# thawro/pytorch-human-pose

Measured on AMD Instinct MI355X. Metric: images/sec (fwd+decode) HigherHRNet-W32 512px, higher is better.
Workload: dtype bf16; 1 GPU; HigherHRNet-W32 inference bf16, batch 32 @ 512x512 per GPU (conv fwd on N(0,1) images + AE decode on constructed maps, 10 people/image, det_thr 0.05, tag_thr 0.5, adjust+refine); global_batch=32, parallelism=image-sharded replicas x1, no data-path collective

## Files before the change

### include/hhrnet.h

```cpp
#ifndef HHRNET_H
#define HHRNET_H
#include <stdint.h>

#ifdef __cplusplus
extern "C" {
#endif

#define HH_ABI_VERSION 3
#define HH_DTYPE_BF16 1
#define HH_DTYPE_FP8 2

typedef struct hh_net hh_net;
typedef struct hh_decoder hh_decoder;

int hh_abi_version(void);
const char *hh_last_error(void);

hh_net *hh_create(int num_kpts, int C, int dtype);
void hh_destroy(hh_net *net);

hh_net *hh_create_classifier(int C, int num_classes, int dtype);
int hh_forward_classifier(hh_net *net, const float *images, int B, int H, int W, float *logits, void *stream);

int hh_num_params(const hh_net *net);
// ... 5 lines not shown

int hh_calibrate(hh_net *net, const float *images, int B, int H, int W, int rounds, void *stream);

int hh_e4m3_encode(const float *x, int64_t n, unsigned char *out);
int hh_e4m3_decode(const unsigned char *x, int64_t n, float *out);

int hh_reserve(hh_net *net, int B, int H, int W);
int64_t hh_workspace_bytes(const hh_net *net);

int hh_forward(hh_net *net, const float *images, int B, int H, int W, float *init_heatmaps, float *deconv_heatmaps,
               int use_graph, void *stream);

int hh_set_multi_lane(hh_net *net, int enable);

int hh_debug_check_plan(const hh_net *net);

double hh_forward_flops(const hh_net *net, int B, int H, int W);

int hh_profile_enable(hh_net *net, int enable);
int hh_profile_count(const hh_net *net);
int hh_profile_get(hh_net *net, int index, int *cfg, double *flops, double *bytes, float *ms, float *kernel_ms, const char **layer);
int hh_profile_clock(hh_net *net, int index, double *ghz);
int hh_conv_config(int cfg, int out[7]);
int hh_conv_config_double_buffered(int cfg);

int hh_debug_conv_bench(int cfg, int B, int Hin, int Win, int cin, int cout, int with_res, int relu, int iters,
                        float *ms_per_launch, unsigned long long *stamps16, int ref_cfg, float *max_diff);

int hh_debug_bb_bench(int B, int H, int W, int iters, float *ms_per_launch, unsigned long long *stamps64);
int hh_debug_bb_compare(int B, int H, int W, int iters, float *max_diff, float *ms_classic, float *ms_pc);
// ... 97 lines not shown
```

### pytorch-human-pose_amd/_lib.py

```python
from __future__ import annotations

import ctypes as C
import os
import subprocess

_HERE = os.path.dirname(os.path.abspath(__file__))
CSRC = os.path.join(_HERE, "csrc")
SO = os.environ.get("HH_LIB") or os.path.join(CSRC, "libhhrnet.so")
HEADER = os.path.join(os.path.dirname(_HERE), "include", "hhrnet.h")
_lib = None


class HHError(RuntimeError):
    pass


def build(force: bool = False, jobs: int = 8) -> str:
    args = ["make", "-C", CSRC, f"-j{jobs}"]
    if force:
        args.append("-B")
    subprocess.check_call(args, stdout=subprocess.DEVNULL)
    return SO


# ... 36 lines not shown
        "hh_debug_conv_bench": (i32, [i32, i32, i32, i32, i32, i32, i32, i32, i32, C.POINTER(C.c_float), vp, i32, C.POINTER(C.c_float)]),
        "hh_debug_bb_bench": (i32, [i32, i32, i32, i32, C.POINTER(C.c_float), vp]),
        "hh_debug_bb_compare": (i32, [i32, i32, i32, i32, C.POINTER(C.c_float), C.POINTER(C.c_float), C.POINTER(C.c_float)]),
        "hh_debug_bb_cover": (i32, [i32, i32, i32, i32, i32, pi64]),
        "hh_preprocess_u8": (i32, [vp, i32, i32, C.POINTER(C.c_double), vp, i32, i32, C.POINTER(C.c_float), C.POINTER(C.c_float), vp]),
        "hh_preprocess_u8_batch": (i32, [vp, vp, i32, vp, i32, i32, C.POINTER(C.c_float), C.POINTER(C.c_float), vp]),
        "hh_flip_images": (i32, [vp, vp, i32, i32, i32, i32, vp]),
        "hh_flip_merge": (i32, [vp, i64, vp, i64, vp, i64, vp, i64, vp, i32, i32, i32, i32, vp]),
        "hh_decoder_create": (vp, [i32, i32, dbl, dbl]),
        "hh_decoder_destroy": (None, [vp]),
        "hh_decoder_reserve": (i32, [vp, i32, i32, i32, i32]),
        "hh_decoder_set_exact_topk": (i32, [vp, i32]),
        "hh_decode": (i32, [vp, vp, i64, vp, i64, vp, pi64, i32, i32, i32, i32, i32, i32, vp, vp, vp, vp, vp]),
        "hh_parse": (i32, [vp, vp, vp, i32, i32, i32, i32, i32, i32, vp, vp, vp, vp, vp]),
        "hh_debug_check_plan": (i32, [vp]),
        "hh_loss_heatmaps": (i32, [vp, i64, vp, vp, i32, i32, i32, i32, vp, vp, i64, vp, vp]),
        "hh_loss_ae_grouping": (i32, [vp, i64, vp, vp, i32, i32, i32, i32, i32, vp, vp, i64, C.c_float, C.c_float, vp, vp]),
        "hh_conv2d_workspace_bytes": (i64, [i32, i32, i32, i32]),
        "hh_conv2d": (i32, [vp, i32, i32, i32, i32, vp, i32, i32, i32, i32, i32, i32, vp, vp, i32, vp, vp, vp]),
        "hh_conv2d_wgrad_workspace_bytes": (i64, [i32, i32, i32, i32, i32, i32, i32]),
        "hh_conv2d_wgrad": (i32, [vp, vp, i32, i32, i32, i32, i32, i32, i32, i32, i32, vp, vp, vp]),
        "hh_fusion_sum_forward": (i32, [vp, vp, i32, i32, i32, i32, i32, i32, vp, vp]),
        "hh_fusion_sum_backward": (i32, [vp, vp, i32, i32, i32, i32, i32, vp, vp, vp, i32, vp]),
        "hh_bn_train_forward": (i32, [vp, i64, i32, vp, vp, C.c_float, vp, i32, vp, vp, vp, vp, vp]),
        "hh_bn_train_backward": (i32, [vp, vp, vp, i64, i32, vp, vp, vp, i32, vp, vp, vp, vp, vp, vp]),
        "hh_bn_train_backward_plain": (i32, [vp, vp, i64, i32, vp, vp, vp, vp, i32, vp, vp, vp, vp, vp]),
        "hh_conv2d_packed_elems": (i64, [i32, i32, i32, i32, i32]),
        "hh_pack_conv_weights_batch": (i32, [i32, vp, vp, vp, vp, vp]),
        "hh_conv2d_packed": (i32, [vp, i32, i32, i32, i32, vp, i32, i32, i32, i32, i32, i32, vp, vp, i32, vp, vp]),
        "hh_bn_train_stats": (i32, [vp, i64, i32, vp, vp, vp]),
# ... 54 lines not shown
```

### pytorch-human-pose_amd/csrc/capi.cpp

```cpp
#include <cmath>
#include <cstring>
#include <string>
#include <vector>

#include "../../include/hhrnet.h"
#include "engine.h"

const char *hh_get_error();
int hh_tap_read_impl(hh_net *n, int index, float *host);

extern "C" {

int hh_abi_version(void) { return HH_ABI_VERSION; }
const char *hh_last_error(void) { return hh_get_error(); }

hh_net *hh_create(int num_kpts, int C, int dtype)
{
    if (dtype != HH_DTYPE_BF16 && dtype != HH_DTYPE_FP8) { hh_set_error("hh_create: dtype must be HH_DTYPE_BF16 or HH_DTYPE_FP8"); return nullptr; }
    if (num_kpts <= 0 || num_kpts > 64 || C <= 0 || C % 16) { hh_set_error("hh_create: need 0 < num_kpts <= 64 and C % 16 == 0"); return nullptr; }
    hh_net *n = new hh_net();
    n->K = num_kpts; n->C = C; n->dtype = dtype;
    n->sw = PlanSwitches::from_env();
    n->build();
    return n;
// ... 85 lines not shown
const char *hh_tap_name(const hh_net *net, int i) { return (i >= 0 && i < (int)net->taps.size()) ? net->taps[i].name.c_str() : nullptr; }
int hh_tap_shape(const hh_net *net, int i, int64_t shape[4])
{
    if (i < 0 || i >= (int)net->taps.size()) return 1;
    const TensorDesc &d = net->tensors[net->taps[i].tensor];
    shape[0] = net->lastB; shape[1] = net->taps[i].C; shape[2] = net->lastH >> d.shift; shape[3] = net->lastW >> d.shift;
    return 0;
}
int hh_tap_read(hh_net *net, int index, float *host_nchw) { return hh_tap_read_impl(net, index, host_nchw); }

int hh_debug_check_plan(const hh_net *net)
{
    std::string why;
    if (net->check_plan(&why)) { hh_set_error("schedule hazard: " + why); return 1; }
    return 0;
}

int hh_profile_enable(hh_net *net, int enable) { net->prof_enabled = enable != 0; net->prof_clk = enable == 2; net->prof_used = 0; return 0; }
int hh_profile_count(const hh_net *net) { return (int)net->prof_used; }
int hh_profile_get(hh_net *net, int i, int *cfg, double *flops, double *bytes, float *ms, float *kernel_ms, const char **layer)
{
    if (i < 0 || i >= (int)net->prof_used) { hh_set_error("hh_profile_get: index out of range"); return 1; }
    const ProfRecord &r = net->prof[i];
    HH_CHECK_HIP(hipEventSynchronize(r.e1));
    HH_CHECK_HIP(hipEventElapsedTime(ms, r.e0, r.e1));
    *cfg = r.cfg; *flops = r.flops; *bytes = r.bytes;
    *layer = net->layers[net->ops[r.op].layer].conv.c_str();
    *kernel_ms = -1.f;
    if (r.slot >= 0 && net->prof_clk && net->d_clk && net->clk_khz > 0) {
        unsigned long long t[2];
// ... 681 lines not shown
```

### pytorch-human-pose_amd/csrc/conv_mfma.hip

```cpp
#include "kernels.h"

#include <utility>

typedef __bf16 bf16x8 __attribute__((ext_vector_type(8)));
typedef __bf16 bf16x2 __attribute__((ext_vector_type(2)));
typedef float f32x16 __attribute__((ext_vector_type(16)));
typedef float f32x2 __attribute__((ext_vector_type(2)));
typedef unsigned u32x4 __attribute__((ext_vector_type(4)));

typedef short i16x2 __attribute__((ext_vector_type(2)));
__device__ __forceinline__ unsigned pack_bf16x2(float a, float b, i16x2 floor)
{
    f32x2 f = {a, b};
    const i16x2 v = __builtin_bit_cast(i16x2, __builtin_convertvector(f, bf16x2));
    return __builtin_bit_cast(unsigned, __builtin_elementwise_max(v, floor));
}
__device__ __forceinline__ float bf16_lo(unsigned u) { return __builtin_bit_cast(float, u << 16); }
__device__ __forceinline__ float bf16_hi(unsigned u) { return __builtin_bit_cast(float, u & 0xffff0000u); }

template <typename F, int... I>
__device__ __forceinline__ void static_for_impl(F &&f, std::integer_sequence<int, I...>)
{
    (f(std::integral_constant<int, I>{}), ...);
}
template <int N, typename F>
__device__ __forceinline__ void static_for(F &&f)
{
    static_for_impl(f, std::make_integer_sequence<int, N>{});
}

#ifdef HH_CONV_DEBUG
__device__ long long g_conv_dbg[8192 * 8];
#define CONV_STAMP(i) do { if (threadIdx.x == 0 && blockIdx.x < 8192) g_conv_dbg[blockIdx.x * 8 + (i)] = (long long)__builtin_readcyclecounter(); } while (0)
#else
#define CONV_STAMP(i)
#endif
template <int KS, int S, int KC, int NT, int WC, int PT, int TW, int DB>
__global__ __launch_bounds__(256, 2) void conv_mfma_kernel(const ConvParams p)
{
    constexpr int RPT = 32 / TW;
    constexpr int WP = 4 / WC;
    constexpr int TH = WP * PT * RPT;
    constexpr int PH = (TH - 1) * S + KS, PW = (TW - 1) * S + KS;
    constexpr int PS = KC * 2 + 16;
    constexpr int C8 = KC / 8;
    constexpr int COUT_T = 32 * NT * WC;
    constexpr int PATCH_BYTES = (PH * PW * PS + 15) & ~15;
    constexpr int P_UNITS = PH * PW * C8;
    constexpr int W_UNITS = KS * KS * C8 * COUT_T;
    constexpr int NPL = (P_UNITS + 255) / 256, NWL = (W_UNITS + 255) / 256, NL = NPL + NWL;
    constexpr int NSTEP = KS * KS * (KC / 16);
    constexpr int LPS = (NL + NSTEP - 1) / NSTEP;
    constexpr int DUMP_OFF = PATCH_BYTES + W_UNITS * 16;
    constexpr int BUF_BYTES = DUMP_OFF + (DB ? 256 * 16 : 0);
// ... 122 lines not shown
#pragma unroll
            for (int pt = 0; pt < PT; ++pt) {
                const int oy = oy0 + (wp * PT + pt) * RPT + dy, ox = ox0 + dx;
                const bool valid = oy < p.Ho && ox < p.Wo;
                const size_t pix = valid ? ((size_t)b * p.Hob + (oy * p.osy + ooy)) * p.Wob + (ox * p.osx + oox) : 0;
#pragma unroll
                for (int nt = 0; nt < NT; ++nt)
#pragma unroll
                    for (int m = 0; m < 2; ++m) {
                        const int c0 = cg * COUT_T + (wc * NT + nt) * 32 + 16 * m + 8 * h;
                        const bool ok = valid && c0 < p.cout_store;
                        const u32x4 v = *reinterpret_cast<const u32x4 *>(p.res + pix * p.res_cs + p.res_coff + (ok ? c0 : 0));
                        rv[pt][nt][m] = ok ? v : u32x4{0u, 0u, 0u, 0u};
                    }
            }
        }
#pragma unroll
        for (int pt = 0; pt < PT; ++pt)
#pragma unroll
            for (int nt = 0; nt < NT; ++nt)
#pragma unroll
                for (int m = 0; m < 2; ++m) {
                    unsigned x0 = 0, x1 = 0, y0 = 0, y1 = 0;
                    if (p.res) {
                        auto s0 = __builtin_amdgcn_permlane32_swap(rv[pt][nt][m][0], rv[pt][nt][m][2], false, false);
                        auto s1 = __builtin_amdgcn_permlane32_swap(rv[pt][nt][m][1], rv[pt][nt][m][3], false, false);
                        x0 = s0[0]; y0 = s0[1]; x1 = s1[0]; y1 = s1[1];
                    }
                    const float4 ba = bs[nt][2 * m], bb = bs[nt][2 * m + 1];
                    acc[nt][pt][8 * m + 0] = ba.x + bf16_lo(x0); acc[nt][pt][8 * m + 1] = ba.y + bf16_hi(x0);
// ... 216 lines not shown
    X(3, 1, 16, 2, 1, 2, 32, 1)  \
    X(3, 1, 16, 2, 1, 1, 16, 1)

#define CFG_ROW(ks, s, kc, nt, wc, pt, tw, db) {ks, s, kc, nt, wc, pt, tw, db},
static const ConvConfig g_configs[] = {CONV_CONFIGS(CFG_ROW)};
#undef CFG_ROW

typedef void (*conv_fn)(const ConvParams);
#define CFG_FN(ks, s, kc, nt, wc, pt, tw, db) conv_mfma_kernel<ks, s, kc, nt, wc, pt, tw, db>,
static const conv_fn g_fns[] = {CONV_CONFIGS(CFG_FN)};
#undef CFG_FN

int conv_num_configs() { return (int)(sizeof(g_configs) / sizeof(g_configs[0])); }
const ConvConfig &conv_config(int i) { return g_configs[i]; }

hipError_t conv_init()
{
    for (int i = 0; i < conv_num_configs(); ++i) {
        hipError_t e = hipFuncSetAttribute(reinterpret_cast<const void *>(g_fns[i]),
                                           hipFuncAttributeMaxDynamicSharedMemorySize, (int)g_configs[i].lds_bytes());
        if (e != hipSuccess) return e;
    }
    return hipSuccess;
}

hipError_t conv_launch(int cfg_index, const ConvParams &p, hipStream_t stream)
{
    const ConvConfig &c = g_configs[cfg_index];
    const unsigned tiles = (unsigned)p.B * p.tiles_y * p.tiles_x, sf = (unsigned)p.ncg * (p.nphase > 1 ? p.nphase : 1);
    const unsigned grid = sf > 1 ? (tiles + 7) / 8 * 8 * sf : tiles;
    HH_LAUNCH(g_fns[cfg_index], dim3(grid), dim3(256), c.lds_bytes(), stream, p);
    return hipGetLastError();
}
```

### pytorch-human-pose_amd/csrc/engine.cpp

```cpp
#include "engine.h"

#include <cmath>
#include <cstdlib>
#include <cstring>

static thread_local std::string g_err;
LaunchProbe &hh_launch_probe()
{
    static thread_local LaunchProbe p;
    return p;
}
void hh_set_error(const std::string &msg) { g_err = msg; }
const char *hh_get_error() { return g_err.c_str(); }

PlanSwitches PlanSwitches::from_env()
{
    auto on = [](const char *name) { const char *v = getenv(name); return v && *v && strcmp(v, "0"); };
    auto is = [](const char *name, const char *val) { const char *v = getenv(name); return v && !strcmp(v, val); };
    PlanSwitches s;
    s.bb32_tile = is("HH_BB32", "tile");
    s.no_bb64 = on("HH_NO_BB64");
    s.no_bb_fp8 = on("HH_NO_BB_FP8");
    s.no_stem_fused = on("HH_NO_STEM_FUSED");
    s.no_junc_pair = on("HH_NO_JUNC_PAIR");
    s.full_join = on("HH_FULL_JOIN");
    s.no_fusion_merge = on("HH_NO_FUSION_MERGE");
    s.no_fused_upsum = on("HH_NO_FUSED_UPSUM");
    s.poison_ws = on("HH_POISON_WS");
    s.poison_lds = on("HH_POISON_LDS");
    s.no_head_fold = on("HH_NO_HEAD_FOLD");
    s.no_conv_db = on("HH_NO_CONV_DB");
    s.no_final_fuse = on("HH_NO_FINAL_FUSE");
    s.keep_waits = on("HH_KEEP_WAITS");
    s.event_system_fence = on("HH_EVENT_SYSTEM_FENCE");
    s.bb_tall = on("HH_NO_BB_TALL") ? 0 : is("HH_BB_TALL", "always") ? 2 : 1;
    if (const char *fc = getenv("HH_FAT_CUS")) { s.fat_cus = s.fat_cus64 = atoi(fc); if (const char *c2 = strchr(fc, ',')) s.fat_cus64 = atoi(c2 + 1); }
    if (const char *sk = getenv("HH_DEBUG_SKIP")) {
        static const struct { const char *name; unsigned bit; } cats[] = {{"s2big", SK_S2BIG}, {"s2", SK_S2}, {"upadd", SK_UPADD}, {"c1x1", SK_C1X1},
            {"c256", SK_C256}, {"c128", SK_C128}, {"junc", SK_JUNC}, {"bb32", SK_BB32}, {"bb64", SK_BB64}, {"stem", SK_STEM}, {"deconv", SK_DECONV},
            {"head", SK_HEAD}, {"trans0", SK_TRANS0}, {"upsum", SK_UPSUM}};
        std::string v = std::string(",") + sk + ",";
        for (const auto &c : cats)
// ... 324 lines not shown
                    auto need_all = [&]() { for (int j = 0; j < nsc; ++j) need(j); };
                    if (i == 0 && n.dtype != 2 && w[0] == 32 && !n.sw.no_fused_upsum) {
                        Op o;
                        o.kind = OP_UPSUM; o.in = x[0]; o.out = OUT; o.C = w[0]; o.relu = 1; o.lane = lane;
                        for (int j = 1; j < nsc; ++j) {
                            const std::string lp = fp + ".scales_fusion_layers.0." + std::to_string(j);
                            o.up[o.nup] = x[j]; o.up_shift[o.nup] = j;
                            o.up_layer[o.nup] = L(lp + ".0", lp + ".1", w[j], w[0], 1, 1);
                            ++o.nup;
                        }
                        o.layer = o.up_layer[0];
                        need_all();
                        n.ops.push_back(o);
                        continue;
                    }
                    Op up;
                    up.kind = OP_UPADD; up.in = x[i]; up.out = OUT; up.C = w[i]; up.relu = (i == 0); up.lane = lane;
                    for (int j = i + 1; j < nsc; ++j) {
                        const std::string lp = fp + ".scales_fusion_layers." + std::to_string(i) + "." + std::to_string(j);
                        const int u = T(w[i], 2 + j);
                        need(j);
                        cb(lp, "0", "1", w[j], w[i], 1, 1, x[j], u, 0);
                        up.up[up.nup] = u; up.up_shift[up.nup] = j - i; ++up.nup;
                    }
                    if (up.nup) { need_all(); n.ops.push_back(up); cur = OUT; }
                    if (i >= 2 && n.dtype != 2 && !n.sw.no_fusion_merge) {
                        int srcs[3] = {-1, -1, -1};
                        ConvLayer ml;
                        ml.cout = w[i]; ml.ks = 3; ml.stride = 2; ml.cin = 0;
                        int tins[3] = {-1, -1, -1};
                        for (int j = 0; j < i; ++j) {
                            const std::string lp = fp + ".scales_fusion_layers." + std::to_string(i) + "." + std::to_string(j);
                            int tin = x[j];
// ... 7 lines not shown
                            tins[j] = tin;
                        }
                        for (int j = i - 1; j >= 0; --j) {
                            const std::string lp = fp + ".scales_fusion_layers." + std::to_string(i) + "." + std::to_string(j);
                            srcs[i - 1 - j] = tins[j];
                            ml.mconv.push_back(lp + "." + std::to_string(i - j - 1) + ".0");
                            ml.mbn.push_back(lp + "." + std::to_string(i - j - 1) + ".1");
                            ml.mcin.push_back(w[j]);
                            ml.cin += w[j];
                        }
                        ml.conv = ml.mconv[0]; ml.bn = ml.mbn[0];
                        n.layers.push_back(ml);
                        need_all();
                        Op &o = conv((int)n.layers.size() - 1, srcs[0], OUT, 1, cur);
                        o.in2 = srcs[1]; o.in3 = srcs[2];
                        cur = OUT;
                        continue;
                    }
                    for (int j = 0; j < i; ++j) {
                        const std::string lp = fp + ".scales_fusion_layers." + std::to_string(i) + "." + std::to_string(j);
                        int tin = x[j];
                        need(j);
                        for (int k = 0; k < i - j - 1; ++k) {
                            const int tmp = T(w[j], 2 + j + k + 1);
                            cb(lp + "." + std::to_string(k), "0", "1", w[j], w[j], 3, 2, tin, tmp, 1);
                            tin = tmp;
                        }
                        need_all();
                        cb(lp + "." + std::to_string(i - j - 1), "0", "1", w[j], w[i], 3, 2, tin, OUT, j == i - 1, cur);
                        cur = OUT;
                    }
                }
                lane = 0;
                if (!last)
                    for (int i = 0; i < nout; ++i) std::swap(x[i], f[i]);
                for (int i = 0; i < nout; ++i)
                    tap("stages." + std::to_string(s) + ".blocks." + std::to_string(2 * b + 1) + "#" + std::to_string(i),
                        last ? CAT : x[i], w[i]);
            }
            if (s < 3) {
                const std::string q = sp + ".transition_layer.transition_blocks." + std::to_string(nsc);
                x[nsc] = T(w[nsc], 2 + nsc);
                if (!n.sw.full_join) { mark(nsc + 1); waitl(nsc, nsc - 1); }
                else join(nsc + 1);
// ... 495 lines not shown
            const TensorDesc &ti = tensors[op.in];
            if (pool_cap < B * op.C) {
                if (d_pool) hipFree(d_pool);
                HH_CHECK_HIP(hipMalloc((void **)&d_pool, (size_t)B * op.C * 4));
                pool_cap = B * op.C;
            }
            HH_CHECK_HIP(launch_avgpool(ti.ptr, ti.C, d_pool, B, (H >> ti.shift) * (W >> ti.shift), op.C, s));
            break;
        }
        case OP_LINEAR:
            HH_CHECK_HIP(launch_linear(d_pool, d_fc_w, d_fc_b, o1, B, 2048, num_classes, s));
            break;
        case OP_STEM: rc = enqueue_stem(op, images, B, H, W, s); break;
        case OP_UPADD: rc = dtype == 2 ? enqueue_fp8_upadd(op, B, H, W, s) : enqueue_upadd(op, B, H, W, s); break;
        case OP_UPSUM: rc = enqueue_upsum(op, B, H, W, s); break;
        case OP_JUNC: rc = enqueue_junc(op, B, H, W, s); break;
        case OP_BB: rc = dtype == 2 ? enqueue_fp8_bb(op, B, H, W, s) : enqueue_bb(op, B, H, W, o2, multi, s, &fin_done); break;
        case OP_QUANT: rc = enqueue_fp8_quant(op, B, H, W, s); break;
        case OP_CONV: rc = dtype == 2 && !op.hi ? enqueue_fp8_conv(op, B, H, W, o1, o2, s) : enqueue_conv(op, B, H, W, o1, o2, s); break;
        }
        if (rc) return 1;
    }
    if (multi)
        for (int l = 1; l < lc.open; ++l)
            if ((lc.dep(0, l) || sw.keep_waits) && lane_wait(0, l)) return 1;
    return 0;
}

int hh_net::prof_record(const Op &op, int cfg, const OpCost &c, unsigned long long **clk)
{
// ... 112 lines not shown
        const ConvLayer &lf = layers[ops[op.fin].layer];
        p.fin_w = lf.d_wfin; p.fin_b = lf.d_bias; p.fin_out = o2; p.fin_K = lf.cout;
        if (lf.d_wfin && bbpc_final_supported(p)) *fin_done = op.fin;
        else { p.fin_w = nullptr; p.fin_b = nullptr; p.fin_out = nullptr; p.fin_K = 0; }
    }
    const int cfg = l1.cout == 64 ? HH_CFG_BB64_FUSED : HH_CFG_BB_FUSED;
    if (prof_enabled && prof_record(op, cfg, op_cost(op, B, H, W, p.fin_out != nullptr), &p.clk)) return 1;
    auto budget = [&](int want) { return !(multi && op.siblings) ? num_cus : want > 0 ? (want < num_cus ? want : num_cus) : (num_cus + 1) / 2; };
    const int fat = budget(sw.fat_cus), fat64 = budget(sw.fat_cus64);
    if (l1.cout == 64) HH_CHECK_HIP(bb64_fused_launch(p, fat64, s));
    else if (!sw.bb32_tile && bbpc_supported(p)) HH_CHECK_HIP(bbpc_launch(p, fat, s));
    else HH_CHECK_HIP(bb_fused_launch(p, num_cus, s));
    return 0;
}

int hh_net::enqueue_conv(const Op &op, int B, int H, int W, float *o1, float *o2, hipStream_t s)
{
    const ConvLayer &l = layers[op.layer];
    const TensorDesc &ti = tensors[op.in];
    ConvParams p{};
    hh_conv_geometry(p, l, op, B, H >> ti.shift, W >> ti.shift, o1, o2);
    p.in = dtype == 2 ? ti.ptr16 : ti.ptr; p.in_cs = ti.C; p.in_coff = op.in_coff;
    p.w = l.d_w; p.bias = l.d_bias;
    if (op.out >= 0) {
        const TensorDesc &to = tensors[op.out];
        p.out = dtype == 2 ? to.ptr16 : to.ptr; p.out_cs = to.C; p.out_coff = op.out_coff;
    }
    if (op.res >= 0) {
        const TensorDesc &tr = tensors[op.res];
        p.res = dtype == 2 ? tr.ptr16 : tr.ptr; p.res_cs = tr.C; p.res_coff = op.res_coff;
    }
    if (op.in2 >= 0) {
        const TensorDesc &t2 = tensors[op.in2];
        if (t2.C != ti.C || t2.shift != ti.shift || (op.in3 >= 0 && (tensors[op.in3].C != ti.C || tensors[op.in3].shift != ti.shift))) {
            hh_set_error("merged fusion conv: inputs differ in shape or pixel stride");
            return 1;
        }
        p.nch0 = l.mcin[0] / l.KC;
        p.nch1 = l.mcin[1] / l.KC;
        p.src_delta1 = t2.ptr - (ti.ptr + op.in_coff);
        if (op.in3 >= 0) p.src_delta2 = tensors[op.in3].ptr - (ti.ptr + op.in_coff);
    }
    p.cout_store = op.cout_store >= 0 ? op.cout_store : round_up(l.cout, 8);
    const int cfg = hh_pick_config(l.ks, l.stride, l.KC, l.NT, p.Wo, l.db);
    const ConvConfig &c = conv_config(cfg);
    p.tiles_x = (p.Wo + c.TW - 1) / c.TW;
    p.tiles_y = (p.Ho + c.th() - 1) / c.th();
    if (prof_enabled && prof_record(op, cfg, op_cost(op, B, H, W), &p.clk)) return 1;
    HH_CHECK_HIP(conv_launch(cfg, p, s));
    return 0;
}

int hh_net::forward(const float *images, int B, int H, int W, float *o1, float *o2, int use_graph, hipStream_t s)
{
    if (!finalized) { hh_set_error("hh_forward: call hh_finalize first"); return 1; }
    if (dtype == 2 && !calibrated) { hh_set_error("hh_forward: fp8 handle without activation scales, call hh_calibrate first"); return 1; }
    if (B > rB || H > rH || W > rW || !ws_ready || (taps_enabled && !taps.empty() && !taps[0].copy))
        if (reserve(B, H, W)) return 1;
    lastB = B; lastH = H; lastW = W;
    if (!use_graph || s == nullptr || taps_enabled || prof_enabled || sw.poison_lds || sw.debug_skip || multi_lane)
        return enqueue(images, B, H, W, o1, o2, s);
    for (auto &g : graphs)
        if (g.images == images && g.o1 == o1 && g.o2 == o2 && g.B == B && g.H == H && g.W == W) {
            HH_CHECK_HIP(hipGraphLaunch(g.exec, s));
// ... 28 lines not shown
    for (size_t i = 0; i < ops.size(); ++i) {
        const Op &op = ops[i];
        if (op.kind == OP_JOIN) { lc.join(op.nlanes); continue; }
        if (op.kind == OP_DEP) { lc.dep(op.lane, op.dep_from); continue; }
        if (op.kind == OP_MARK) { lc.set_mark(op.dep_from, op.nlanes); continue; }
        if (op.kind == OP_WAITL) {
            if (!lc.marked[op.dep_from]) { if (why) *why = "op " + std::to_string(i) + " waits for a lane the last mark did not record"; return 1; }
            lc.wait_mark(op.lane, op.dep_from);
            continue;
        }
        const int l = op.lane;
        if (l >= lc.open) { if (why) *why = "op " + std::to_string(i) + " runs on a lane that was never forked"; return 1; }
        std::vector<int> rd, wr;
        switch (op.kind) {
        case OP_CONV: rd = {op.in, op.res, op.in2, op.in3}; wr = {op.out}; break;
        case OP_UPADD: case OP_UPSUM: rd = {op.in, op.up[0], op.up[1], op.up[2]}; wr = {op.out}; break;
        case OP_BB: rd = {op.in}; wr = {op.out}; break;
        case OP_JUNC: rd = {op.in, op.in2, op.res, op.in3}; wr = {op.out, op.out2}; break;
        case OP_STEM: wr = {op.out}; break;
        case OP_QUANT: rd = {op.out}; wr = {op.out}; break;
        case OP_TAP: continue;
        case OP_AVGPOOL: rd = {op.in}; break;
        default: break;
        }
        const int t = lc.launch(l);
        for (int x : rd) {
            if (x < 0) continue;
            if (!before(writer[x], l)) {
                if (why) *why = "RAW: op " + std::to_string(i) + " (lane " + std::to_string(l) + ") reads tensor " + std::to_string(x) +
                                " written by op " + std::to_string(writer[x].op) + " (lane " + std::to_string(writer[x].lane) + ") without an edge";
// ... 53 lines not shown
    case OP_BB: {
        const TensorDesc &ti = tensors[op.in], &to = tensors[op.out];
        const double Cb = layers[op.layer].cout, npix = (double)B * (H >> ti.shift) * (W >> ti.shift);
        c.flops = 2.0 * 2.0 * npix * Cb * Cb * 9.0;
        if (dtype == 2)
            c.bytes = (2.0 + (ti.b16 ? 2.0 : 0.0) + (to.b16 ? 2.0 : 0.0)) * npix * Cb + 2.0 * 9 * Cb * Cb;
        else
            c.bytes = 2.0 * npix * Cb * 2 + 2.0 * 2 * 9 * Cb * Cb;
        if (fin) {
            const double K2 = layers[ops[op.fin].layer].cout;
            c.flops += op_cost(ops[op.fin], B, H, W).flops;
            c.bytes += (4.0 * K2 - 2.0 * Cb) * npix + 2.0 * Cb * K2;
        }
        break;
    }
    case OP_CONV: {
        const ConvLayer &l = layers[op.layer];
        const TensorDesc &ti = tensors[op.in];
        const int hin = H >> ti.shift, win = W >> ti.shift, ho = l.stride == 2 ? hin / 2 : hin, wo = l.stride == 2 ? win / 2 : win;
        const int nph = l.transposed && l.py < 0 ? 4 : 1;
        const double acin = l.acct_cin ? l.acct_cin : l.cin;
        const double opix = (double)B * ho * wo * nph;
        const bool e4m3 = dtype == 2 && !op.hi;
        double out_e = 0, res_e = 0;
        if (op.out >= 0) out_e = e4m3 ? (tensors[op.out].f8 ? 1 : 0) + (tensors[op.out].b16 ? 2 : 0) : 2;
        if (op.res >= 0) res_e = e4m3 && !tensors[op.res].b16 ? 1 : 2;
        c.flops = 2.0 * opix * acin * l.cout * l.ks * l.ks;
        c.bytes = (e4m3 ? 1.0 : 2.0) * ((double)B * hin * win * acin + acin * l.cout * l.ks * l.ks * nph) +
                  (out_e + res_e + (op.f32_out ? 4 : 0)) * opix * l.cout;
        break;
    }
    default:
        break;
    }
    return c;
}

double hh_net::flops(int B, int H, int W) const
{
    double f = kind == 1 ? 2.0 * B * 2048.0 * num_classes : 0.0;
    for (const Op &op : ops) f += op_cost(op, B, H, W).flops;
    return f;
}

// ... 47 lines not shown
```

### pytorch-human-pose_amd/csrc/engine.h

```cpp
#pragma once
#include <map>
#include <string>
#include <vector>

#include "kernels.h"

void hh_set_error(const std::string &msg);
void hh_pack_weights(const float *W, const float *scale, int ks, int cin, int cout, int KC, int COUT_T, bool transposed,
                     int py, int px, std::vector<unsigned short> &packed);
#define HH_CHECK_HIP(expr)                                                                             \
    do {                                                                                               \
        hipError_t _e = (expr);                                                                        \
        if (_e != hipSuccess) {                                                                        \
            hh_set_error(std::string(#expr) + ": " + hipGetErrorString(_e));                           \
            return 1;                                                                                  \
        }                                                                                              \
    } while (0)

struct ParamSlot {
    std::string name;
    std::vector<int64_t> shape;
    std::vector<float> data;
    bool loaded = false;
    bool counter = false;
// ... 20 lines not shown
    bf16_raw *d_wfin = nullptr;
    std::vector<float> w_scale;
    float *d_mult = nullptr;
};

struct TensorDesc {
    int C = 0, shift = 0;
    bf16_raw *ptr = nullptr;
    bool f8 = true, b16 = false;
    bf16_raw *ptr16 = nullptr;
    bool zero_init = false;
    int ones_channel = -1;
    bool shared_scale = false;
};

enum OpKind { OP_CONV, OP_UPADD, OP_TAP, OP_BB, OP_JOIN, OP_AVGPOOL, OP_LINEAR, OP_DEP, OP_JUNC, OP_STEM, OP_MARK, OP_WAITL, OP_QUANT, OP_UPSUM };

struct Op {
    OpKind kind = OP_CONV;
    int layer = -1, layer2 = -1;
    int layer3 = -1;
    int layer4 = -1;
    int in2 = -1, out2 = -1;
    int in3 = -1;
    int in = -1, in_coff = 0;
    int out = -1, out_coff = 0;
    int res = -1, res_coff = 0;
    int relu = 0;
    int f32_out = 0;
    int cout_store = -1;
    int scatter = 0;
// ... 32 lines not shown
    const void *images;
    void *o1, *o2;
    int B, H, W;
    hipGraphExec_t exec;
};

struct PlanSwitches {
    bool bb32_tile = false;
    bool no_bb64 = false;
    bool no_bb_fp8 = false;
    bool no_stem_fused = false;
    bool no_junc_pair = false;
    bool full_join = false;
    bool no_fusion_merge = false;
    bool no_fused_upsum = false;
    bool poison_ws = false;
    int fat_cus = 0, fat_cus64 = 0;
    bool event_system_fence = false;
    bool keep_waits = false;
    bool no_final_fuse = false;
    int bb_tall = 1;
    bool no_conv_db = false;
    bool no_head_fold = false;
    bool poison_lds = false;
    unsigned debug_skip = 0;
    bool fp8_trunk8 = false;
    bool fp8_heads8 = false;
    static PlanSwitches from_env();
};

enum SkipCat { SK_S2BIG = 1, SK_S2 = 2, SK_UPADD = 4, SK_C1X1 = 8, SK_C256 = 16, SK_C128 = 32, SK_JUNC = 64, SK_BB32 = 128, SK_BB64 = 256,
               SK_STEM = 512, SK_DECONV = 1024, SK_HEAD = 2048, SK_TRANS0 = 4096, SK_UPSUM = 8192 };
inline unsigned hh_skip_cats(const Op &op, const std::vector<ConvLayer> &layers, const std::vector<TensorDesc> &tensors)
{
    switch (op.kind) {
    case OP_UPADD: return SK_UPADD;
    case OP_UPSUM: return SK_UPSUM;
    case OP_JUNC: return SK_JUNC;
    case OP_STEM: return SK_STEM;
    case OP_BB: return layers[op.layer].cout == 32 ? SK_BB32 : layers[op.layer].cout == 64 ? SK_BB64 : 0;
    case OP_CONV: break;
    default: return 0;
    }
    const ConvLayer &l = layers[op.layer];
    if (l.transposed) return SK_DECONV;
    if (op.f32_out) return SK_HEAD;
    if (l.stride == 2) return SK_S2 | (l.cin >= 128 ? SK_S2BIG : 0) | (l.cin == 256 && l.mconv.empty() && tensors[op.in].shift == 2 ? SK_TRANS0 : 0);
    if (l.ks == 1) return SK_C1X1;
    if (l.cin == 256 && l.cout == 256) return SK_C256;
    if (l.cin == 128 && l.cout == 128) return SK_C128;
    if (l.cin == 256 && tensors[op.in].shift == 2) return SK_TRANS0;
    return 0;
}

struct OpCost { double flops = 0, bytes = 0; };

// ... 43 lines not shown
    int add_param(const std::string &name, std::vector<int64_t> shape, bool counter = false);
    int finalize();
    int reserve(int B, int H, int W);
    int enqueue(const float *images, int B, int H, int W, float *o1, float *o2, hipStream_t s);
    int forward(const float *images, int B, int H, int W, float *o1, float *o2, int use_graph, hipStream_t s);
    double flops(int B, int H, int W) const;
    OpCost op_cost(const Op &op, int B, int H, int W, bool fin = false) const;
    int prof_record(const Op &op, int cfg, const OpCost &c, unsigned long long **clk);
    float bn_fold(const std::string &bn, int co, const float *cb, float *shift) const;
    void fold_layer(const ConvLayer &l, int coutp, std::vector<float> &scale, std::vector<float> &shift) const;
    int enqueue_stem(const Op &op, const float *images, int B, int H, int W, hipStream_t s);
    int enqueue_upadd(const Op &op, int B, int H, int W, hipStream_t s);
    int enqueue_upsum(const Op &op, int B, int H, int W, hipStream_t s);
    int enqueue_junc(const Op &op, int B, int H, int W, hipStream_t s);
    int enqueue_bb(const Op &op, int B, int H, int W, float *o2, bool multi, hipStream_t s, int *fin_done);
    int enqueue_conv(const Op &op, int B, int H, int W, float *o1, float *o2, hipStream_t s);
    int finalize_fp8();
    int calibrate(const float *images, int B, int H, int W, int rounds, hipStream_t s);
    int resolve_scales();
    int enqueue_fp8_conv(const Op &op, int B, int H, int W, float *o1, float *o2, hipStream_t s);
    int enqueue_fp8_upadd(const Op &op, int B, int H, int W, hipStream_t s);
    int enqueue_fp8_quant(const Op &op, int B, int H, int W, hipStream_t s);
    void assign_fp8_formats();
    int enqueue_fp8_bb(const Op &op, int B, int H, int W, hipStream_t s);
    void release_workspace();
    ~hh_net();
};

int hh_family_pick(int ks, int stride, int cin_pad, int coutp, int *KC, int *NT);
int hh_pick_config(int ks, int stride, int KC, int NT, int Wo, int db = 0);

// ... 31 lines not shown
```

### pytorch-human-pose_amd/csrc/kernels.h

```cpp
#pragma once
#include <hip/hip_runtime.h>
#include <stdint.h>

#include <hip/hip_ext.h>

typedef uint16_t bf16_raw;

struct LaunchProbe { hipEvent_t start = nullptr, stop = nullptr; };
LaunchProbe &hh_launch_probe();
#define HH_LAUNCH(kernel, grid, block, lds, stream, ...)                                                            \
    do {                                                                                                            \
        LaunchProbe &lp_ = hh_launch_probe();                                                                       \
        if (lp_.start) {                                                                                            \
            hipExtLaunchKernelGGL(kernel, grid, block, lds, stream, lp_.start, lp_.stop, 0, __VA_ARGS__);           \
            lp_ = LaunchProbe{};                                                                                    \
        } else {                                                                                                    \
            hipLaunchKernelGGL(kernel, grid, block, lds, stream, __VA_ARGS__);                                      \
        }                                                                                                           \
    } while (0)

struct ConvParams {
    const bf16_raw *in;
    int in_cs, in_coff;
    int Hin, Win;
    const bf16_raw *w;
    const float *bias;
    const bf16_raw *res;
    int res_cs, res_coff;
    bf16_raw *out;
    int out_cs, out_coff;
    float *out_f32;
    int Hob, Wob;
    int osy, ooy, osx, oox;
    int Ho, Wo;
    int cin;
    int cout_real, cout_store;
    int relu;
    int pad_y, pad_x;
    int B, tiles_x, tiles_y, ncg;
    int nphase;
    size_t phase_stride;
    unsigned long long *stamps;
    unsigned long long *clk;
    int nch0, nch1;
    ptrdiff_t src_delta1, src_delta2;
};

struct ConvConfig {
    int KS, S, KC, NT, WC, PT, TW;
    int DB;
    int cout_t() const { return 32 * NT * WC; }
    int th() const { return (4 / WC) * PT * (32 / TW); }
    size_t lds_bytes() const {
        int PH = (th() - 1) * S + KS, PW = (TW - 1) * S + KS;
        size_t patch = ((size_t)PH * PW * (KC * 2 + 16) + 15) & ~(size_t)15;
        const size_t buf = patch + (size_t)KS * KS * KC * cout_t() * 2;
        return DB ? 2 * (buf + 256 * 16) : buf;
    }
};

int conv_num_configs();
const ConvConfig &conv_config(int i);
hipError_t conv_launch(int cfg_index, const ConvParams &p, hipStream_t stream);
hipError_t conv_init();

struct Fp8ConvParams {
    const unsigned char *in;
    int in_cs, in_coff;
    int Hin, Win;
    const unsigned char *w;
    const float *mult;
    const float *bias;
    const unsigned char *res;
    int res_cs, res_coff;
    float res_scale;
    const bf16_raw *res16;
    int res16_cs, res16_coff;
    unsigned char *out;
    int out_cs, out_coff;
// ... 251 lines not shown
```

Before: 7023 images/sec.

## Fuse lower-resolution 1x1 upsample branches into the stride-2 fusion conv epilogue

Adds an OP_DOWNSUM op and a templated UP variant of the MFMA conv kernel. For HRNet fusion outputs at scale i>=1, the kernel computes the 1x1 convs of coarser branches (j>i) per tile into LDS and adds their nearest-upsampled values into the stride-2 conv epilogue before the store. This removes separate upadd launches and the intermediate tensor round trips through memory. In exchange it uses more LDS and registers per block, may lower occupancy, and repeats some 1x1 work per conv channel group.

```diff
diff --git a/include/hhrnet.h b/include/hhrnet.h
--- a/include/hhrnet.h
+++ b/include/hhrnet.h
@@ -43,6 +43,7 @@
 int hh_set_multi_lane(hh_net *net, int enable);
 
 int hh_debug_check_plan(const hh_net *net);
+int hh_debug_count_ops(const hh_net *net, const char *kind);
 
 double hh_forward_flops(const hh_net *net, int B, int H, int W);
 
diff --git a/pytorch-human-pose_amd/_lib.py b/pytorch-human-pose_amd/_lib.py
--- a/pytorch-human-pose_amd/_lib.py
+++ b/pytorch-human-pose_amd/_lib.py
@@ -74,6 +74,7 @@
         "hh_decode": (i32, [vp, vp, i64, vp, i64, vp, pi64, i32, i32, i32, i32, i32, i32, vp, vp, vp, vp, vp]),
         "hh_parse": (i32, [vp, vp, vp, i32, i32, i32, i32, i32, i32, vp, vp, vp, vp, vp]),
         "hh_debug_check_plan": (i32, [vp]),
+        "hh_debug_count_ops": (i32, [vp, cp]),
         "hh_loss_heatmaps": (i32, [vp, i64, vp, vp, i32, i32, i32, i32, vp, vp, i64, vp, vp]),
         "hh_loss_ae_grouping": (i32, [vp, i64, vp, vp, i32, i32, i32, i32, i32, vp, vp, i64, C.c_float, C.c_float, vp, vp]),
         "hh_conv2d_workspace_bytes": (i64, [i32, i32, i32, i32]),
diff --git a/pytorch-human-pose_amd/csrc/capi.cpp b/pytorch-human-pose_amd/csrc/capi.cpp
--- a/pytorch-human-pose_amd/csrc/capi.cpp
+++ b/pytorch-human-pose_amd/csrc/capi.cpp
@@ -123,6 +123,22 @@
     std::string why;
     if (net->check_plan(&why)) { hh_set_error("schedule hazard: " + why); return 1; }
     return 0;
+}
+
+int hh_debug_count_ops(const hh_net *net, const char *kind)
+{
+    static const struct { const char *name; OpKind k; } kinds[] = {{"conv", OP_CONV}, {"upadd", OP_UPADD}, {"upsum", OP_UPSUM}, {"downsum", OP_DOWNSUM},
+                                                                   {"bb", OP_BB}, {"junc", OP_JUNC}, {"stem", OP_STEM}};
+    const bool all = !strcmp(kind, "launch");
+    int n = 0, known = all;
+    for (const auto &e : kinds) {
+        if (!all && strcmp(kind, e.name)) continue;
+        known = 1;
+        for (const Op &op : net->ops) n += op.kind == e.k;
+    }
+    if (all)
+        for (const Op &op : net->ops) n += (op.kind == OP_AVGPOOL || op.kind == OP_LINEAR || op.kind == OP_QUANT) - (op.kind == OP_BB && op.fin >= 0);
+    return known ? n : -1;
 }
 
 int hh_profile_enable(hh_net *net, int enable) { net->prof_enabled = enable != 0; net->prof_clk = enable == 2; net->prof_used = 0; return 0; }
diff --git a/pytorch-human-pose_amd/csrc/conv_mfma.hip b/pytorch-human-pose_amd/csrc/conv_mfma.hip
--- a/pytorch-human-pose_amd/csrc/conv_mfma.hip
+++ b/pytorch-human-pose_amd/csrc/conv_mfma.hip
@@ -1,5 +1,6 @@
 #include "kernels.h"
 
+#include <type_traits>
 #include <utility>
 
 typedef __bf16 bf16x8 __attribute__((ext_vector_type(8)));
@@ -35,9 +36,60 @@
 #else
 #define CONV_STAMP(i)
 #endif
-template <int KS, int S, int KC, int NT, int WC, int PT, int TW, int DB>
-__global__ __launch_bounds__(256, 2) void conv_mfma_kernel(const ConvParams p)
-{
+constexpr int UP_PS = 144;
+constexpr int UP_BYTES = 40 * UP_PS;
+constexpr int UP_BATCH = 8;
+__device__ __forceinline__ unsigned pack2(float a, float b)
+{
+    f32x2 f = {a, b};
+    return __builtin_bit_cast(unsigned, __builtin_convertvector(f, bf16x2));
+}
+template <int TH, int TW>
+__device__ __forceinline__ void up_source_tile(const FusionDownParams &d, int j, int ct, int cg, int b, int oy0, int ox0, int Ho, int Wo,
+                                               char *lds_u, int lane)
+{
+    const int sh = d.shift[j], FW = TW >> sh, NPX = (TH >> sh) * FW;
+    const int r = lane & 31, h = lane >> 5;
+    const int Hj = Ho >> sh, Wj = Wo >> sh;
+    const int gy = (oy0 >> sh) + r / FW, gx = (ox0 >> sh) + r % FW;
+    const bool ok = r < NPX && gy < Hj && gx < Wj;
+    const bf16_raw *src = d.src[j] + ((size_t)b * Hj * Wj + (ok ? (size_t)gy * Wj + gx : 0)) * d.src_cs[j] + 8 * h;
+    const int nstep = d.nstep[j];
+    const u32x4 *w = reinterpret_cast<const u32x4 *>(d.w[j]) + ((size_t)cg * nstep * 2 + h) * 64 + ct * 32 + r;
+    f32x16 acc;
+    const float *bias = d.bias[j] + cg * 64 + ct * 32;
+    static_for<4>([&](auto gc) {
+        constexpr int g = decltype(gc)::value;
+        const float4 bv = *reinterpret_cast<const float4 *>(bias + 8 * g + 4 * h);
+        const float z = __builtin_bit_cast(float, 0u);
+        acc[4 * g + 0] = bv.x + z; acc[4 * g + 1] = bv.y + z; acc[4 * g + 2] = bv.z + z; acc[4 * g + 3] = bv.w + z;
+    });
+    for (int s0 = 0; s0 < nstep; s0 += UP_BATCH) {
+        u32x4 fa[UP_BATCH], fb[UP_BATCH];
+        static_for<UP_BATCH>([&](auto sc) {
+            constexpr int s = decltype(sc)::value;
+            fa[s] = w[128 * (s0 + s)];
+            fb[s] = *reinterpret_cast<const u32x4 *>(src + 16 * (s0 + s));
+        });
+        static_for<UP_BATCH>([&](auto sc) {
+            constexpr int s = decltype(sc)::value;
+            acc = __builtin_amdgcn_mfma_f32_32x32x16_bf16(__builtin_bit_cast(bf16x8, fa[s]), __builtin_bit_cast(bf16x8, fb[s]), acc, 0, 0, 0);
+        });
+    }
+    if (r < NPX) {
+        const i16x2 id = {(short)-32768, (short)-32768};
+        unsigned *dst = reinterpret_cast<unsigned *>(lds_u + r * UP_PS + (ct * 32 + 4 * h) * 2);
+        static_for<4>([&](auto gc) {
+            constexpr int g = decltype(gc)::value;
+            *reinterpret_cast<uint2 *>(dst + 4 * g) = make_uint2(pack_bf16x2(acc[4 * g + 0], acc[4 * g + 1], id), pack_bf16x2(acc[4 * g + 2], acc[4 * g + 3], id));
+        });
+    }
+}
+
+template <int KS, int S, int KC, int NT, int WC, int PT, int TW, int DB, int UP = 0>
+__global__ __launch_bounds__(256, 2) void conv_mfma_kernel(const std::conditional_t<UP != 0, ConvUpParams, ConvParams> p)
+{
+    static_assert(!UP || (NT == 2 && WC == 1 && PT == 1 && !DB), "UP: 64-cout tile, one wave per pixel row tile");
     constexpr int RPT = 32 / TW;
     constexpr int WP = 4 / WC;
     constexpr int TH = WP * PT * RPT;
@@ -190,6 +242,32 @@
                         rv[pt][nt][m] = ok ? v : u32x4{0u, 0u, 0u, 0u};
                     }
             }
+        }
+        if constexpr (UP) {
+            const FusionDownParams &d = p.up;
+            char *lds_u = smem + BUF_BYTES;
+            if ((wave >> 1) < d.nsrc)
+                up_source_tile<TH, TW>(d, wave >> 1, wave & 1, cg, b, oy0, ox0, p.Ho, p.Wo, lds_u + (wave >> 1) * 32 * UP_PS, lane);
+            __syncthreads();
+            const int ly = wp * RPT + dy;
+#pragma unroll
+            for (int nt = 0; nt < NT; ++nt)
+#pragma unroll
+                for (int m = 0; m < 2; ++m) {
+                    const u32x4 bv = rv[0][nt][m];
+                    float v[8] = {bf16_lo(bv[0]), bf16_hi(bv[0]), bf16_lo(bv[1]), bf16_hi(bv[1]),
+                                  bf16_lo(bv[2]), bf16_hi(bv[2]), bf16_lo(bv[3]), bf16_hi(bv[3])};
+#pragma unroll
+                    for (int j = 0; j < 2; ++j)
+                        if (j < d.nsrc) {
+                            const int sh = d.shift[j];
+                            const u32x4 uv = *reinterpret_cast<const u32x4 *>(lds_u + (j * 32 + (ly >> sh) * (TW >> sh) + (dx >> sh)) * UP_PS +
+                                                                              (nt * 32 + 16 * m + 8 * h) * 2);
+                            v[0] += bf16_lo(uv[0]); v[1] += bf16_hi(uv[0]); v[2] += bf16_lo(uv[1]); v[3] += bf16_hi(uv[1]);
+                            v[4] += bf16_lo(uv[2]); v[5] += bf16_hi(uv[2]); v[6] += bf16_lo(uv[3]); v[7] += bf16_hi(uv[3]);
+                        }
+                    rv[0][nt][m] = u32x4{pack2(v[0], v[1]), pack2(v[2], v[3]), pack2(v[4], v[5]), pack2(v[6], v[7])};
+                }
         }
 #pragma unroll
         for (int pt = 0; pt < PT; ++pt)
@@ -436,14 +514,40 @@
 int conv_num_configs() { return (int)(sizeof(g_configs) / sizeof(g_configs[0])); }
 const ConvConfig &conv_config(int i) { return g_configs[i]; }
 
+typedef void (*conv_up_fn)(const ConvUpParams);
+static conv_up_fn fusion_down_fn(const ConvConfig &c)
+{
+    if (c.KS != 3 || c.S != 2 || c.KC != 16 || c.NT != 2 || c.WC != 1 || c.PT != 1 || c.DB) return nullptr;
+    return c.TW == 32 ? conv_mfma_kernel<3, 2, 16, 2, 1, 1, 32, 0, 1> : c.TW == 16 ? conv_mfma_kernel<3, 2, 16, 2, 1, 1, 16, 0, 1> : nullptr;
+}
+bool fusion_down_supported(int cfg_index) { return fusion_down_fn(g_configs[cfg_index]) != nullptr; }
+size_t fusion_down_lds_bytes(int cfg_index) { return g_configs[cfg_index].lds_bytes() + UP_BYTES; }
+
 hipError_t conv_init()
 {
     for (int i = 0; i < conv_num_configs(); ++i) {
         hipError_t e = hipFuncSetAttribute(reinterpret_cast<const void *>(g_fns[i]),
                                            hipFuncAttributeMaxDynamicSharedMemorySize, (int)g_configs[i].lds_bytes());
         if (e != hipSuccess) return e;
+        if (conv_up_fn fu = fusion_down_fn(g_configs[i])) {
+            e = hipFuncSetAttribute(reinterpret_cast<const void *>(fu), hipFuncAttributeMaxDynamicSharedMemorySize, (int)fusion_down_lds_bytes(i));
+            if (e != hipSuccess) return e;
+        }
     }
     return hipSuccess;
+}
+
+hipError_t fusion_down_launch(int cfg_index, const ConvUpParams &p, hipStream_t stream)
+{
+    const FusionDownParams &d = p.up;
+    const conv_up_fn fn = fusion_down_fn(g_configs[cfg_index]);
+    if (!fn || !p.res || p.nphase > 1 || d.nsrc < 1 || d.nsrc > 2) return hipErrorInvalidValue;
+    for (int j = 0; j < d.nsrc; ++j)
+        if (d.nstep[j] <= 0 || d.nstep[j] % UP_BATCH || d.shift[j] != j + 1) return hipErrorInvalidValue;
+    const unsigned tiles = (unsigned)p.B * p.tiles_y * p.tiles_x;
+    const unsigned grid = p.ncg > 1 ? (tiles + 7) / 8 * 8 * p.ncg : tiles;
+    HH_LAUNCH(fn, dim3(grid), dim3(256), fusion_down_lds_bytes(cfg_index), stream, p);
+    return hipGetLastError();
 }
 
 hipError_t conv_launch(int cfg_index, const ConvParams &p, hipStream_t stream)
diff --git a/pytorch-human-pose_amd/csrc/engine.cpp b/pytorch-human-pose_amd/csrc/engine.cpp
--- a/pytorch-human-pose_amd/csrc/engine.cpp
+++ b/pytorch-human-pose_amd/csrc/engine.cpp
@@ -26,6 +26,7 @@
     s.full_join = on("HH_FULL_JOIN");
     s.no_fusion_merge = on("HH_NO_FUSION_MERGE");
     s.no_fused_upsum = on("HH_NO_FUSED_UPSUM");
+    s.no_fused_downsum = on("HH_NO_FUSED_DOWNSUM");
     s.poison_ws = on("HH_POISON_WS");
     s.poison_lds = on("HH_POISON_LDS");
     s.no_head_fold = on("HH_NO_HEAD_FOLD");
@@ -380,9 +381,23 @@
                         n.ops.push_back(o);
                         continue;
                     }
+                    Op pend;
+                    if (i >= 1 && n.dtype != 2 && w[1] % 64 == 0 && !n.sw.no_fused_downsum)
+                        for (int j = i + 1; j < nsc; ++j) {
+                            const std::string lp = fp + ".scales_fusion_layers." + std::to_string(i) + "." + std::to_string(j);
+                            pend.up[pend.nup] = x[j]; pend.up_shift[pend.nup] = j - i;
+                            pend.up_layer[pend.nup] = L(lp + ".0", lp + ".1", w[j], w[i], 1, 1);
+                            ++pend.nup;
+                        }
+                    auto take_up = [&](Op &o) {
+                        if (!pend.nup) return;
+                        o.kind = OP_DOWNSUM; o.nup = pend.nup;
+                        for (int k = 0; k < pend.nup; ++k) { o.up[k] = pend.up[k]; o.up_shift[k] = pend.up_shift[k]; o.up_layer[k] = pend.up_layer[k]; }
+                        pend.nup = 0;
+                    };
                     Op up;
                     up.kind = OP_UPADD; up.in = x[i]; up.out = OUT; up.C = w[i]; up.relu = (i == 0); up.lane = lane;
-                    for (int j = i + 1; j < nsc; ++j) {
+                    for (int j = i + 1; j < nsc && !pend.nup; ++j) {
                         const std::string lp = fp + ".scales_fusion_layers." + std::to_string(i) + "." + std::to_string(j);
                         const int u = T(w[i], 2 + j);
                         need(j);
@@ -420,6 +435,7 @@
                         need_all();
                         Op &o = conv((int)n.layers.size() - 1, srcs[0], OUT, 1, cur);
                         o.in2 = srcs[1]; o.in3 = srcs[2];
+                        take_up(o);
                         cur = OUT;
                         continue;
                     }
@@ -433,7 +449,7 @@
                             tin = tmp;
                         }
                         need_all();
-                        cb(lp + "." + std::to_string(i - j - 1), "0", "1", w[j], w[i], 3, 2, tin, OUT, j == i - 1, cur);
+                        take_up(cb(lp + "." + std::to_string(i - j - 1), "0", "1", w[j], w[i], 3, 2, tin, OUT, j == i - 1, cur));
                         cur = OUT;
                     }
                 }
@@ -959,6 +975,7 @@
         case OP_STEM: rc = enqueue_stem(op, images, B, H, W, s); break;
         case OP_UPADD: rc = dtype == 2 ? enqueue_fp8_upadd(op, B, H, W, s) : enqueue_upadd(op, B, H, W, s); break;
         case OP_UPSUM: rc = enqueue_upsum(op, B, H, W, s); break;
+        case OP_DOWNSUM: rc = enqueue_downsum(op, B, H, W, s); break;
         case OP_JUNC: rc = enqueue_junc(op, B, H, W, s); break;
         case OP_BB: rc = dtype == 2 ? enqueue_fp8_bb(op, B, H, W, s) : enqueue_bb(op, B, H, W, o2, multi, s, &fin_done); break;
         case OP_QUANT: rc = enqueue_fp8_quant(op, B, H, W, s); break;
@@ -1101,11 +1118,10 @@
     return 0;
 }
 
-int hh_net::enqueue_conv(const Op &op, int B, int H, int W, float *o1, float *o2, hipStream_t s)
+int hh_net::conv_params(const Op &op, int B, int H, int W, float *o1, float *o2, ConvParams &p, int *cfg_out)
 {
     const ConvLayer &l = layers[op.layer];
     const TensorDesc &ti = tensors[op.in];
-    ConvParams p{};
     hh_conv_geometry(p, l, op, B, H >> ti.shift, W >> ti.shift, o1, o2);
     p.in = dtype == 2 ? ti.ptr16 : ti.ptr; p.in_cs = ti.C; p.in_coff = op.in_coff;
     p.w = l.d_w; p.bias = l.d_bias;
@@ -1133,8 +1149,39 @@
     const ConvConfig &c = conv_config(cfg);
     p.tiles_x = (p.Wo + c.TW - 1) / c.TW;
     p.tiles_y = (p.Ho + c.th() - 1) / c.th();
+    *cfg_out = cfg;
+    return 0;
+}
+
+int hh_net::enqueue_conv(const Op &op, int B, int H, int W, float *o1, float *o2, hipStream_t s)
+{
+    ConvParams p{};
+    int cfg = -1;
+    if (conv_params(op, B, H, W, o1, o2, p, &cfg)) return 1;
     if (prof_enabled && prof_record(op, cfg, op_cost(op, B, H, W), &p.clk)) return 1;
     HH_CHECK_HIP(conv_launch(cfg, p, s));
+    return 0;
+}
+
+int hh_net::enqueue_downsum(const Op &op, int B, int H, int W, hipStream_t s)
+{
+    ConvUpParams p{};
+    int cfg = -1;
+    if (conv_params(op, B, H, W, nullptr, nullptr, p, &cfg)) return 1;
+    const ConvLayer &lc = layers[op.layer];
+    bool fits = op.res >= 0 && op.out >= 0 && op.nup >= 1 && op.nup <= 2 && fusion_down_supported(cfg) && lc.cout % 64 == 0;
+    for (int j = 0; j < op.nup && fits; ++j) {
+        const ConvLayer &l = layers[op.up_layer[j]];
+        const TensorDesc &t = tensors[op.up[j]];
+        fits = t.shift == tensors[op.res].shift + j + 1 && op.up_shift[j] == j + 1 && l.KC == 32 && l.NT == 2 && l.ncg == lc.ncg &&
+               l.cout == lc.cout && l.cin % 64 == 0 && l.cin <= t.C;
+        p.up.src[j] = t.ptr; p.up.src_cs[j] = t.C; p.up.shift[j] = j + 1; p.up.nstep[j] = l.cin / 16;
+        p.up.w[j] = l.d_w; p.up.bias[j] = l.d_bias;
+    }
+    if (!fits) { hh_set_error("plan: fusion output does not fit the UP form of conv_mfma.hip (HH_NO_FUSED_DOWNSUM=1)"); return 1; }
+    p.up.nsrc = op.nup;
+    if (prof_enabled && prof_record(op, HH_CFG_FUSION_DOWN, op_cost(op, B, H, W), &p.clk)) return 1;
+    HH_CHECK_HIP(fusion_down_launch(cfg, p, s));
     return 0;
 }
 
@@ -1193,6 +1240,7 @@
         std::vector<int> rd, wr;
         switch (op.kind) {
         case OP_CONV: rd = {op.in, op.res, op.in2, op.in3}; wr = {op.out}; break;
+        case OP_DOWNSUM: rd = {op.in, op.res, op.in2, op.in3, op.up[0], op.up[1]}; wr = {op.out}; break;
         case OP_UPADD: case OP_UPSUM: rd = {op.in, op.up[0], op.up[1], op.up[2]}; wr = {op.out}; break;
         case OP_BB: rd = {op.in}; wr = {op.out}; break;
         case OP_JUNC: rd = {op.in, op.in2, op.res, op.in3}; wr = {op.out, op.out2}; break;
@@ -1276,7 +1324,7 @@
         }
         break;
     }
-    case OP_CONV: {
+    case OP_CONV: case OP_DOWNSUM: {
         const ConvLayer &l = layers[op.layer];
         const TensorDesc &ti = tensors[op.in];
         const int hin = H >> ti.shift, win = W >> ti.shift, ho = l.stride == 2 ? hin / 2 : hin, wo = l.stride == 2 ? win / 2 : win;
@@ -1290,6 +1338,13 @@
         c.flops = 2.0 * opix * acin * l.cout * l.ks * l.ks;
         c.bytes = (e4m3 ? 1.0 : 2.0) * ((double)B * hin * win * acin + acin * l.cout * l.ks * l.ks * nph) +
                   (out_e + res_e + (op.f32_out ? 4 : 0)) * opix * l.cout;
+        for (int j = 0; j < op.nup && op.kind == OP_DOWNSUM; ++j) {
+            const ConvLayer &lu = layers[op.up_layer[j]];
+            const TensorDesc &t = tensors[op.up[j]];
+            const double npix = (double)B * (H >> t.shift) * (W >> t.shift);
+            c.flops += 2.0 * npix * lu.cin * lu.cout;
+            c.bytes += 2.0 * npix * lu.cin + 2.0 * lu.cin * lu.cout;
+        }
         break;
     }
     default:
diff --git a/pytorch-human-pose_amd/csrc/engine.h b/pytorch-human-pose_amd/csrc/engine.h
--- a/pytorch-human-pose_amd/csrc/engine.h
+++ b/pytorch-human-pose_amd/csrc/engine.h
@@ -58,7 +58,7 @@
     bool shared_scale = false;
 };
 
-enum OpKind { OP_CONV, OP_UPADD, OP_TAP, OP_BB, OP_JOIN, OP_AVGPOOL, OP_LINEAR, OP_DEP, OP_JUNC, OP_STEM, OP_MARK, OP_WAITL, OP_QUANT, OP_UPSUM };
+enum OpKind { OP_CONV, OP_UPADD, OP_TAP, OP_BB, OP_JOIN, OP_AVGPOOL, OP_LINEAR, OP_DEP, OP_JUNC, OP_STEM, OP_MARK, OP_WAITL, OP_QUANT, OP_UPSUM, OP_DOWNSUM };
 
 struct Op {
     OpKind kind = OP_CONV;
@@ -121,6 +121,7 @@
     bool full_join = false;
     bool no_fusion_merge = false;
     bool no_fused_upsum = false;
+    bool no_fused_downsum = false;
     bool poison_ws = false;
     int fat_cus = 0, fat_cus64 = 0;
     bool event_system_fence = false;
@@ -146,7 +147,7 @@
     case OP_JUNC: return SK_JUNC;
     case OP_STEM: return SK_STEM;
     case OP_BB: return layers[op.layer].cout == 32 ? SK_BB32 : layers[op.layer].cout == 64 ? SK_BB64 : 0;
-    case OP_CONV: break;
+    case OP_CONV: case OP_DOWNSUM: break;
     default: return 0;
     }
     const ConvLayer &l = layers[op.layer];
@@ -220,7 +221,9 @@
     int enqueue_upsum(const Op &op, int B, int H, int W, hipStream_t s);
     int enqueue_junc(const Op &op, int B, int H, int W, hipStream_t s);
     int enqueue_bb(const Op &op, int B, int H, int W, float *o2, bool multi, hipStream_t s, int *fin_done);
+    int conv_params(const Op &op, int B, int H, int W, float *o1, float *o2, ConvParams &p, int *cfg);
     int enqueue_conv(const Op &op, int B, int H, int W, float *o1, float *o2, hipStream_t s);
+    int enqueue_downsum(const Op &op, int B, int H, int W, hipStream_t s);
     int finalize_fp8();
     int calibrate(const float *images, int B, int H, int W, int rounds, hipStream_t s);
     int resolve_scales();
diff --git a/pytorch-human-pose_amd/csrc/kernels.h b/pytorch-human-pose_amd/csrc/kernels.h
--- a/pytorch-human-pose_amd/csrc/kernels.h
+++ b/pytorch-human-pose_amd/csrc/kernels.h
@@ -19,6 +19,15 @@
         }                                                                                                           \
     } while (0)
 
+struct FusionDownParams {
+    const bf16_raw *src[2];
+    int src_cs[2];
+    int shift[2];
+    int nstep[2];
+    const bf16_raw *w[2];
+    const float *bias[2];
+    int nsrc;
+};
 struct ConvParams {
     const bf16_raw *in;
     int in_cs, in_coff;
@@ -45,6 +54,7 @@
     int nch0, nch1;
     ptrdiff_t src_delta1, src_delta2;
 };
+struct ConvUpParams : ConvParams { FusionDownParams up; };
 
 struct ConvConfig {
     int KS, S, KC, NT, WC, PT, TW;
@@ -63,6 +73,10 @@
 const ConvConfig &conv_config(int i);
 hipError_t conv_launch(int cfg_index, const ConvParams &p, hipStream_t stream);
 hipError_t conv_init();
+#define HH_CFG_FUSION_DOWN 108
+bool fusion_down_supported(int cfg_index);
+size_t fusion_down_lds_bytes(int cfg_index);
+hipError_t fusion_down_launch(int cfg_index, const ConvUpParams &p, hipStream_t stream);
 
 struct Fp8ConvParams {
     const unsigned char *in;
```

Result: no change. 7073 images/sec (median of 6 runs) (+0.7%).
